# drowe67/radae

Measured on AMD Instinct MI355X. Metric: vocoder-feature frames/sec (enc+chan+dec), model19, higher is better.
Workload: dtype f32 I/O, 2xf16 (22-bit) MFMA operands, f32 accumulate (refine: f64 MFMA)

## Files before the change

### radae_amd/csrc/rade_dev.h

```cpp
#ifndef RADE_DEV_H
#define RADE_DEV_H

#include <stdint.h>

#ifdef __cplusplus
extern "C" {
#endif

#define RD_M        160
#define RD_NCP      32
#define RD_SYM      192
#define RD_NC       30
#define RD_NS       4
#define RD_NMF      960
#define RD_NEOO     1152
#define RD_RXBUF    2112
#define RD_NFC      40
#define RD_NQ       16
#define RD_NTAP     101
#define RD_NINMAX   1120
#define RD_LATENT   80
#define RD_ZMF      240
#define RD_FEAT_MF  432
#define RD_NEOOBITS 180
// ... 94 lines not shown

#define RD_EF_KB   (RD_ENC_W / 16)
#define RD_EF_TILE (RD_EF_KB * 1024)
typedef struct {
    const unsigned short *xf; int NQ;
    int B, T, K0, K1, dil;
    const unsigned short *Wp16; const float *Wscale; const float *bias; int N, act;
    float *y; long y_sb, y_st;
    unsigned short *yf; int ycol;
    int seq_taps, no_pair;
    int pair;
    const float *xin; int Kin; const float *Wp;
} rd_encf_args;
int rd_launch_encf_gemm(const rd_encf_args *a, rd_stream_t s);
int rd_launch_encf_dense1(const rd_encf_args *a, rd_stream_t s);
int rd_launch_encf_hist(unsigned short *xf, int NQ, float *x32, long x32_sb, int B, int T, int dir, rd_stream_t s);

int rd_launch_enc_pack(const float *features, float *xin, int B, int T, rd_stream_t s);
int rd_launch_pad_rows(const float *src, float *dst, long R, int K, int Kpad, rd_stream_t s);
int rd_launch_chan_symbol(const float *z, const float *H, const float *noise, float *out, long n_real, int mode, float p0, float p1, unsigned long long seed, rd_stream_t s);
int rd_launch_carry_rows(float *x, int B, int Tcap, int W, int nhist, int T, const int *n_rows, rd_stream_t s);
int rd_launch_ofdm_mod(const rd_tables *tab, const float *z, void *tx, long tx_stride, int B, int n_mf, int linear, rd_stream_t s);
int rd_launch_ofdm_mod_mp(const rd_tables *tab, const float *z, void *tx, long tx_stride, int B, int n_mf, const void *G, void *mp, double *part, int linear, rd_stream_t s);
int rd_launch_eoo_build(const rd_tables *tab, const float *bits, float *eoo, int B, rd_stream_t s);
int rd_launch_copy_eoo(const float *eoo, void *out, long stride, int B, rd_stream_t s);

enum { RD_IRX_LS = 0, RD_IRX_MEAN6 = 1, RD_IRX_ALL = 2, RD_IRX_NONE = 3 };
typedef struct {
    const rd_tables *tab; const void *rx; long rx_stride;
    const float *foff;
    int n_mf, time_offset, eq, coarse_mag, B;
    float mag_scale;
    float *z_hat;
    double *part;
    const float *z_ref; long long *n_err;
} rd_irx_args;
int rd_launch_irx(const rd_irx_args *a, rd_stream_t s);

// ... 125 lines not shown
```

### radae_amd/csrc/rade_enc.hip

```cpp
#include "rade_devutil.h"

#define EF_TILE RD_EF_TILE

template <bool LIBM_TANH>
__device__ __forceinline__ void encf_emit(const rd_encf_args &a, int b, int t, int ch0, f32x4 v, f32x4 sc, f32x4 bs)
{
#pragma unroll
    for (int c = 0; c < 4; c++) {
        float x = v[c] * sc[c] + bs[c];
        if (a.act == 1) x = clamp1(LIBM_TANH ? tanhf(x) : gate_tanh(x));
        v[c] = x;
    }
    if (a.yf) {
        const int col = a.ycol + ch0;
        _Float16 *o = (_Float16 *)a.yf + ((size_t)b * a.NQ + 1 + (t >> 5)) * EF_TILE + (col >> 4) * 1024 + ((col >> 3) & 1) * 256 + (t & 31) * 8 + (col & 4);
        f16x4 hi, lo;
#pragma unroll
        for (int c = 0; c < 4; c++) { const float x = 256.0f * v[c]; const _Float16 h = (_Float16)x; hi[c] = h; lo[c] = (_Float16)(x - (float)h); }
        *(f16x4 *)o = hi; *(f16x4 *)(o + 512) = lo;
    } else {
        *(f32x4 *)(a.y + (size_t)b * a.y_sb + (size_t)t * a.y_st + ch0) = v;
    }
}

// ... 98 lines not shown
#pragma unroll
        for (int i = 0; i < NT; i++)
#pragma unroll
            for (int g = 0; g < 4; g++) {
                const int ch0 = 32 * (nt0 + i) + 8 * g + 4 * half;
                if (ch0 >= a.N) continue;
                const f32x4 bs = a.bias ? *(const f32x4 *)(a.bias + ch0) : (f32x4){ 0.0f, 0.0f, 0.0f, 0.0f };
                f32x4 sc = { 0x1p-18f, 0x1p-18f, 0x1p-18f, 0x1p-18f };
                if (SINGLE) { sc = *(const f32x4 *)(a.Wscale + ch0); sc *= 0x1p-8f; }
                const f32x4 v = { acc[q][i][4 * g], acc[q][i][4 * g + 1], acc[q][i][4 * g + 2], acc[q][i][4 * g + 3] };
                encf_emit<false>(a, b, t, ch0, v, sc, bs);
            }
    }
}

__global__ __launch_bounds__(64) void k_encf_dense1(rd_encf_args a)
{
    constexpr int NT = 2;
    const int lane = threadIdx.x, r = lane & 31, half = lane >> 5;
    const int tpq = (a.T + 31) >> 5;
    const int b = blockIdx.x / tpq, qt = blockIdx.x - b * tpq;
    const int t = 32 * qt + r;
    const float *p = a.xin + ((size_t)b * a.T + min(t, a.T - 1)) * a.Kin + 4 * half;
    f32x16 acc[NT];
#pragma unroll
    for (int i = 0; i < NT; i++)
#pragma unroll
        for (int j = 0; j < 16; j++) acc[i][j] = 0.0f;
    const float *wp = a.Wp + (size_t)lane * 4;
    const size_t wstep = (size_t)NT * 256;
    const int nkb = a.Kin >> 3;
    f32x4 av = *(const f32x4 *)p;
    f32x4 bv[NT];
#pragma unroll
    for (int i = 0; i < NT; i++) bv[i] = *(const f32x4 *)(wp + i * 256);
    for (int kb = 0; kb < nkb; kb++) {
        f32x4 an = av; f32x4 bn[NT];
#pragma unroll
        for (int i = 0; i < NT; i++) bn[i] = bv[i];
        if (kb + 1 < nkb) {
            an = *(const f32x4 *)(p + (kb + 1) * 8);
#pragma unroll
            for (int i = 0; i < NT; i++) bn[i] = *(const f32x4 *)(wp + wstep + i * 256);
        }
#pragma unroll
        for (int s = 0; s < 4; s++)
#pragma unroll
            for (int i = 0; i < NT; i++)
                acc[i] = __builtin_amdgcn_mfma_f32_32x32x2f32(bv[i][s], av[s], acc[i], 0, 0, 0);
        av = an;
#pragma unroll
        for (int i = 0; i < NT; i++) bv[i] = bn[i];
        wp += wstep;
    }
    if (t >= a.T) return;
#pragma unroll
// ... 43 lines not shown
        }
    }
}

extern "C" int rd_launch_encf_hist(unsigned short *xf, int NQ, float *x32, long x32_sb, int B, int T, int dir, rd_stream_t s)
{
    if (B <= 0) return 0;
    hipLaunchKernelGGL(k_encf_hist, dim3(B), dim3(256), 0, (hipStream_t)s, xf, NQ, x32, x32_sb, T, dir);
    return (int)hipGetLastError();
}

extern "C" int rd_launch_encf_dense1(const rd_encf_args *a, rd_stream_t s)
{
    if (a->B <= 0 || a->T <= 0) return 0;
    if (a->N != 64 || (a->Kin & 7) || !a->yf) return -1;
    hipLaunchKernelGGL(k_encf_dense1, dim3(a->B * ((a->T + 31) >> 5)), dim3(64), 0, (hipStream_t)s, *a);
    return (int)hipGetLastError();
}

extern "C" int rd_launch_encf_gemm(const rd_encf_args *a, rd_stream_t s)
{
    if (a->B <= 0 || a->T <= 0) return 0;
    const int ntt = (a->N + 31) >> 5, tpq = (a->T + 31) >> 5;
    if ((a->K0 & 15) || (a->K1 & 15) || ntt % 3 || (a->N & 3) || a->dil < 0 || a->dil > 2) return -1;
    hipStream_t st = (hipStream_t)s;
    const int seq = a->seq_taps, nopair = a->no_pair;
    rd_encf_args b = *a;
    const int ntile = a->B * tpq;
    b.pair = (ntt == 6 && !nopair) ? 1 : 0;
    const dim3 g = b.pair ? dim3(((ntile + 7) / 8) * 16, 1) : dim3(ntile, ntt / 3), blk(64);
    const bool ti = a->K0 > 0 && a->K0 == a->K1 && !seq;
// ... 9 lines not shown
```

### radae_amd/csrc/rade_engine.c

```c
#define _GNU_SOURCE
#define __HIP_PLATFORM_AMD__ 1
#include <hip/hip_runtime_api.h>

#include <pthread.h>
#include <time.h>
#include <sched.h>
#include <stdio.h>
#include <stdlib.h>
#include <string.h>
#include <stdint.h>
#include <math.h>

#include "rade_batch.h"
#include "rade_api.h"
#include "rade_host.h"

#define CHK(x) do { hipError_t e_ = (x); if (e_ != hipSuccess) { fprintf(stderr, "rade: HIP error %s at %s:%d\n", hipGetErrorString(e_), __FILE__, __LINE__); goto fail; } } while (0)

static int g_engines_open;
double rade_host_cpu_quota(void)
{
    cpu_set_t set; double n = 1.0;
    if (sched_getaffinity(0, sizeof set, &set) == 0) n = (double)CPU_COUNT(&set);
    FILE *f = fopen("/sys/fs/cgroup/cpu.max", "r");
// ... 23 lines not shown

#define ON_DEV(h) do { if (h) (void)hipSetDevice((h)->device); } while (0)

#define RADE_PROF_MAXEV 256
#define RADE_PROF_MAXIV 4096
struct rade_batch {
    struct owned *owned;
    int alloc_failed;
    int B, max_tx_mf, device, flags, trace_cap, Tcap;
    int R, dec_rows;
    int unsync_off_after;
    unsigned short *corrq16, *corra16, *wfwd16, *bpf16; double *vm; int rx_lds, rx_census;
    int feat_in, enc_kpad, bottleneck1;
    float *dec2_x, *dec2_gi, *dec2_hbuf, *dec2_h[5];
    rd_tables *d_tab;
    dev_lin enc_dense1, enc_zdense, dec_dense1, dec_output, enc_gin[5], dec_gin[5], enc_conv[5], dec_conv[5], dec_glu[5];
    float *enc_whh[5], *enc_bhh[5], *dec_whh[5], *dec_bhh[5];
    unsigned short *dec_whq[5]; float *dec_whs[5];
    float *enc_xin, *enc_x, *enc_gi, *enc_h[5], *enc_z, *eoo, *eoo_bits;
    unsigned short *enc_xf; int enc_nq, enc_seq_taps, enc_no_pair;
    int enc_hist_frag;
    int bypass_dec;
    int tx_linear;
    double *irx_part; long irx_part_cap; float *irx_foff; long long *irx_err;
    rd_bpf_state *tx_bpf, *tx_bpf_init; void *tx_raw; float *tx_chain; float *eoo_filt;
    void *chan_scratch; void *chan_mp;
    float *chan_ps, *chan_ps_host;
    float *rs_sigma; double *rs_part, *rs_stats;
    int *loss_len; double *loss_res, *loss_part; long loss_part_cap;
    rd_rx_stream *rx_st; rd_rx_round *rx_round;
// ... 181 lines not shown
    if (h->R < 1) h->R = 1;
    if (h->R > RD_RX_ROUND_MAX) h->R = RD_RX_ROUND_MAX;
    h->dec_rows = getenv("RADE_DEC_ROWS") ? atoi(getenv("RADE_DEC_ROWS")) : 48;
    if (h->dec_rows < 3) h->dec_rows = 3;
    if (h->dec_rows > 63) h->dec_rows = 63;
    const size_t DR = (size_t)h->dec_rows;

    rd_tables *tab = malloc(sizeof *tab);
    rd_tables_fill(tab);
    h->d_tab = dev_upload(h, tab, sizeof *tab);
    h->corrq16 = upload_table16(h, tab, rd_corrq16_table_fill, RD_CORRQ16_HALFS);
    h->corra16 = upload_table16(h, tab, rd_corra16_table_fill, RD_CORRA16_HALFS);
    h->wfwd16 = upload_table16(h, tab, rd_wfwd16_table_fill, RD_WFWD16_HALFS);
    h->bpf16 = upload_table16(h, tab, rd_bpf16_table_fill, RD_BPF16_HALFS);
    free(tab);
    {
        double vm[8][RD_M];
        for (int n = 0; n < RD_M; n++) { const double nu = ((double)n - 79.5) / 80.0; double v = 1.0; for (int m = 0; m < 8; m++) { vm[m][n] = v; v *= nu; } }
        h->vm = dev_upload(h, vm, sizeof vm);
    }
    h->rx_lds = rd_rx_sync_prepare();
    h->rx_census = getenv("RADE_RX2_CENSUS") ? atoi(getenv("RADE_RX2_CENSUS")) : 0;
    if (h->alloc_failed || h->rx_lds <= 0) goto fail;

    int err = 0;
    h->feat_in = m.enc_dense1.n_in; h->enc_kpad = (h->feat_in + 15) & ~15; h->bottleneck1 = (cfg->flags & RADE_BATCH_BOTTLENECK1) != 0;
    err |= upload_lin(h, &h->enc_dense1, m.enc_dense1.w, m.enc_dense1.b, NULL, 64, h->feat_in, h->enc_kpad);
    err |= upload_lin(h, &h->enc_zdense, m.enc_zdense.w, m.enc_zdense.b, NULL, 80, 864, 864);
    err |= upload_lin(h, &h->dec_dense1, m.dec_dense1.w, m.dec_dense1.b, NULL, 96, 80, 80);
    err |= upload_lin(h, &h->dec_output, m.dec_output.w, m.dec_output.b, NULL, h->feat_in, 736, 736);
// ... 65 lines not shown
    h->dec2_gi = dev_zeros(h, sizeof(float) * B * T * 288);
    h->dec2_hbuf = dev_zeros(h, sizeof(float) * B * T * 96);
    h->dtcache = dev_zeros(h, sizeof(float) * B * 2 * RD_NMF * RD_NFC);
    if (h->trace_cap > 0) {
        h->trace = dev_zeros(h, sizeof(rd_rx_trace) * B * h->trace_cap);
        h->trace_z = dev_zeros(h, sizeof(float) * B * h->trace_cap * RD_ZMF);
    }
    h->h_small = must(h, pinned_alloc_opt(h, sizeof(int) * (8 + B * 8)));
    h->lcg_seeds = malloc(sizeof(unsigned) * B);
    for (size_t b = 0; b < B; b++) h->lcg_seeds[b] = 1u;
    h->d_lcg_seeds = dev_upload(h, h->lcg_seeds, sizeof(unsigned) * B);
    if (h->alloc_failed) { fprintf(stderr, "rade: device allocation failed\n"); goto fail; }
    for (int i = 0; i < 2 * RADE_PROF_MAXEV; i++) CHK(hipEventCreate(&h->prof_ev[i]));
    CHK(hipEventCreateWithFlags(&h->ev_block, hipEventBlockingSync | hipEventDisableTiming));
    rade_batch_rx_reset(h);
    if (rd_launch_eoo_build(h->d_tab, NULL, h->eoo, h->B, NULL)) goto fail;
    CHK(hipDeviceSynchronize());
    rd_model_free(&m);
    return h;
fail:
    if (have_model) rd_model_free(&m);
    if (h) rade_batch_close(h);
    return NULL;
}

rade_batch *rade_batch_open(const char *blob_path, const rade_batch_config *cfg)
{
    FILE *f = blob_path ? fopen(blob_path, "rb") : NULL;
    if (!f) { fprintf(stderr, "rade: cannot open weight blob %s\n", blob_path ? blob_path : "(null)"); return NULL; }
    fseek(f, 0, SEEK_END); long n = ftell(f); fseek(f, 0, SEEK_SET);
    void *buf = malloc(n);
// ... 6 lines not shown

void rade_batch_close(rade_batch *h)
{
    if (!h) return;
    ON_DEV(h);
    while (h->owned) disown(h, h->owned->p);
    if (h->ev_block) hipEventDestroy(h->ev_block);
    __atomic_sub_fetch(&g_engines_open, 1, __ATOMIC_RELAXED);
    for (int i = 0; i < 2 * RADE_PROF_MAXEV; i++) if (h->prof_ev[i]) hipEventDestroy(h->prof_ev[i]);
    free(h->lcg_seeds);
    free(h);
}

int rade_batch_n_streams(const rade_batch *h) { return h->B; }
const rd_tables *rd_batch_tables(const rade_batch *h) { return h->d_tab; }
int rd_batch_has_tx_bpf(const rade_batch *h) { return h->tx_bpf != NULL; }

static void prof_drain(rade_batch *h)
{
    for (int i = 0; i < h->prof_cnt; i++) {
        float ms = 0;
        if (hipEventSynchronize(h->prof_ev[2 * i + 1]) == hipSuccess && hipEventElapsedTime(&ms, h->prof_ev[2 * i], h->prof_ev[2 * i + 1]) == hipSuccess) {
            h->prof_ms[h->prof_cls[i]] += ms; h->prof_flops[h->prof_cls[i]] += h->prof_fl[i]; h->prof_n[h->prof_cls[i]]++;
            float t0 = 0;
            if (h->prof_ref && h->iv_n < RADE_PROF_MAXIV && hipEventElapsedTime(&t0, h->prof_ref, h->prof_ev[2 * i]) == hipSuccess) {
                h->iv_cls[h->iv_n] = h->prof_cls[i]; h->iv_t0[h->iv_n] = t0; h->iv_t1[h->iv_n] = t0 + ms; h->iv_n++;
            }
        }
    }
    h->prof_cnt = 0;
// ... 45 lines not shown

static int encf_gemm(rade_batch *h, const dev_lin *w, int K1, int K0, int dil, float *y, long y_sb, long y_st, int ycol, int T, int act, void *stream)
{
    rd_encf_args g;
    memset(&g, 0, sizeof g);
    g.xf = h->enc_xf; g.NQ = h->enc_nq; g.B = h->B; g.T = T; g.K0 = K0; g.K1 = K1; g.dil = dil;
    g.Wp16 = w->wp16; g.Wscale = w->wscale16; g.bias = w->bias; g.N = w->N; g.act = act;
    g.y = y; g.y_sb = y_sb; g.y_st = y_st; if (!y) { g.yf = h->enc_xf; g.ycol = ycol; }
    g.seq_taps = h->enc_seq_taps; g.no_pair = h->enc_no_pair;
    if (K0 + K1 != w->K || !w->wp16) { fprintf(stderr, "rade: internal GEMM shape error (%d+%d != %d)\n", K0, K1, w->K); return -1; }
    PROF_BEGIN(h, stream);
    const int rc = rd_launch_encf_gemm(&g, stream);
    PROF_END(h, stream, RADE_PROF_GEMM, 2.0 * (double)h->B * T * (K0 + K1) * w->N);
    return rc;
}
static int encode_core_frag(rade_batch *h, int T, float *z, void *stream)
{
    const int B = h->B;
    int e = h->enc_hist_frag ? 0 : rd_launch_encf_hist(h->enc_xf, h->enc_nq, h->enc_x, (long)(2 + h->Tcap) * RD_ENC_W, B, T, 0, stream);
    {
        rd_encf_args g;
        memset(&g, 0, sizeof g);
        g.xf = h->enc_xf; g.NQ = h->enc_nq; g.B = B; g.T = T; g.bias = h->enc_dense1.bias; g.N = 64; g.act = 1; g.yf = h->enc_xf; g.ycol = 0;
        g.xin = h->enc_xin; g.Kin = h->enc_kpad; g.Wp = h->enc_dense1.wp;
        PROF_BEGIN(h, stream); e |= rd_launch_encf_dense1(&g, stream); PROF_END(h, stream, RADE_PROF_GEMM, 2.0 * (double)B * T * h->enc_kpad * 64);
    }
    e |= encf_gemm(h, &h->enc_gin[0], ENC_IN[0], 0, 0, h->enc_gi, (long)T * 192, 192, 0, T, 0, stream);
    for (int l = 0; l < 5 && !e; l++) {
        const int in = ENC_IN[l], cin = in + 64;
        rd_scan_args s = { h->enc_gi, (long)T * 192, 192, h->enc_whh[l], h->enc_bhh[l], h->enc_h[l], NULL, 0, 0, NULL, 0, NULL, B, T, 64, h->enc_xf, h->enc_nq, in };
        PROF_BEGIN(h, stream); e |= rd_launch_gru_scan(&s, stream); PROF_END(h, stream, RADE_PROF_SCAN, 2.0 * B * T * 192 * 64);
        e |= encf_gemm(h, &h->enc_conv[l], cin, cin, ENC_DIL[l], NULL, 0, 0, cin, T, 1, stream);
        if (l < 4) e |= encf_gemm(h, &h->enc_gin[l + 1], ENC_IN[l + 1], 0, 0, h->enc_gi, (long)T * 192, 192, 0, T, 0, stream);
        else e |= encf_gemm(h, &h->enc_zdense, 864, 0, 0, z, (long)T * RD_LATENT, RD_LATENT, 0, T, h->bottleneck1 ? 1 : 0, stream);
    }
    e |= rd_launch_encf_hist(h->enc_xf, h->enc_nq, h->enc_x, (long)(2 + h->Tcap) * RD_ENC_W, B, T, 1, stream);
    h->enc_hist_frag = !e;
    return e;
}

static int encode_core(rade_batch *h, int T, float *z, void *stream)
{
    const int B = h->B, W = RD_ENC_W;
    if (h->enc_xf && (long)B * T > 16384) return encode_core_frag(h, T, z, stream);
    h->enc_hist_frag = 0;
    const long xsb = (long)(2 + h->Tcap) * W;
    float *x0 = h->enc_x + 2 * W;
    int e = 0;
    dev_lin d1 = h->enc_dense1; d1.wp16 = NULL; d1.wscale16 = NULL;
    e |= gemm(h, &d1, h->enc_xin, (long)T * h->enc_kpad, h->enc_kpad, h->enc_kpad, NULL, 0, 0, 0, NULL, NULL, x0, xsb, W, B, T, 1, stream);
    for (int l = 0; l < 5 && !e; l++) {
        const int in = ENC_IN[l], cin = in + 64;
        e |= gemm(h, &h->enc_gin[l], x0, xsb, W, in, NULL, 0, 0, 0, NULL, NULL, h->enc_gi, (long)T * 192, 192, B, T, 0, stream);
        rd_scan_args s = { h->enc_gi, (long)T * 192, 192, h->enc_whh[l], h->enc_bhh[l], h->enc_h[l], x0 + in, xsb, W, NULL, 0, NULL, B, T, 64 };
        PROF_BEGIN(h, stream); e |= rd_launch_gru_scan(&s, stream); PROF_END(h, stream, RADE_PROF_SCAN, 2.0 * B * T * 192 * 64);
        e |= gemm(h, &h->enc_conv[l], x0, xsb, W, cin, x0 - (long)ENC_DIL[l] * W, xsb, W, cin, NULL, NULL, x0 + cin, xsb, W, B, T, 1, stream);
    }
    e |= gemm(h, &h->enc_zdense, x0, xsb, W, 864, NULL, 0, 0, 0, NULL, NULL, z, (long)T * RD_LATENT, RD_LATENT, B, T, h->bottleneck1 ? 1 : 0, stream);
    e |= rd_launch_carry_rows(h->enc_x, B, h->Tcap, W, 2, T, NULL, stream);
// ... 3 lines not shown
static int tx_bpf_pass(rade_batch *h, int n, int len0, void *out, long out_stride, void *stream, int advance)
{
    rd_bpf_args ba;
    memset(&ba, 0, sizeof ba);
    ba.state = h->tx_bpf; ba.state_stride = sizeof(rd_bpf_state); ba.len0_const = len0; ba.avail_const = n;
    ba.tab = h->d_tab; ba.bpf16 = h->bpf16; ba.x = h->tx_raw; ba.x_stride = tx_raw_stride(h); ba.y = out; ba.y_stride = out_stride;
    ba.chain = h->tx_chain; ba.chain_stride = h->max_tx_mf + 8; ba.n_blocks = 1 + (n > len0 ? (n - len0 + RD_NMF - 1) / RD_NMF : 0); ba.B = h->B; ba.clip = 1; ba.advance = advance;
    PROF_BEGIN(h, stream);
    const int rc = rd_launch_bpf(&ba, stream);
    PROF_END(h, stream, RADE_PROF_BPF, 8.0 * 101.0 * (double)h->B * n);
    return rc;
}

static int encode_features(rade_batch *h, const float *features_dev, int T, float *z, void *stream)
{
    const int e = rd_launch_enc_pack(features_dev, h->enc_xin, h->B, T, stream);
    return e | encode_core(h, T, z, stream);
}
static int modulate(rade_batch *h, const float *z, int n_mf, void *iq_out, long iq_stride, void *stream)
{
    void *mod_out = h->tx_bpf ? h->tx_raw : iq_out; const long mod_stride = h->tx_bpf ? tx_raw_stride(h) : iq_stride;
    PROF_BEGIN(h, stream);
    int e = rd_launch_ofdm_mod(h->d_tab, z, mod_out, mod_stride, h->B, n_mf, h->tx_linear, stream);
    PROF_END(h, stream, RADE_PROF_MOD, 8.0 * h->B * n_mf * 5 * 30 * 160);
    if (h->tx_bpf) e |= tx_bpf_pass(h, n_mf * RD_NMF, RD_NMF, iq_out, iq_stride, stream, 1);
    return e;
}

int rade_batch_tx(rade_batch *h, const float *features_dev, int n_mf, void *iq_out_dev, long iq_stride, float *z_out_dev, void *stream)
{
    ON_DEV(h);
    if (!h || !features_dev || !iq_out_dev || n_mf <= 0 || n_mf > h->max_tx_mf || h->feat_in != 84) return -1;
    if (misaligned16(z_out_dev)) return -1;
    float *z = z_out_dev ? z_out_dev : h->enc_z;
    int e = encode_features(h, features_dev, 3 * n_mf, z, stream);
    e |= modulate(h, z, n_mf, iq_out_dev, iq_stride, stream);
    return e ? -1 : n_mf * RD_NMF;
}
// ... 119 lines not shown
{
    ON_DEV(h);
    if (!h || !p || n_mf <= 0 || n_mf > h->max_tx_mf || h->feat_in != 84 || p->n_sig != n_mf * RD_NMF || !rx_out_dev || (h->tx_linear && p->with_eoo)) return -1;
    if (!features_dev || misaligned16(p->G_dev)) return -1;
    const float *ps_dev;
    if (chan_streams_upload(h, p, ps, stream, &ps_dev)) return -1;
    if (!p->G_dev || h->tx_bpf) {
        if (!iq_out_dev) return -1;
        if (rade_batch_tx(h, features_dev, n_mf, iq_out_dev, iq_stride, NULL, stream) != p->n_sig) return -1;
        return channel_dev(h, iq_out_dev, iq_stride, rx_out_dev, rx_stride, p, ps_dev, stream);
    }
    if (dev_grow(h, &h->chan_mp, NULL, (long)h->B * h->max_tx_mf * RD_NMF, sizeof(float) * 2, 1)) return -1;
    const int B = h->B;
    int e = encode_features(h, features_dev, 3 * n_mf, h->enc_z, stream);
    PROF_BEGIN(h, stream);
    e |= rd_launch_ofdm_mod_mp(h->d_tab, h->enc_z, iq_out_dev, iq_stride, B, n_mf, p->G_dev, h->chan_mp, (double *)h->chan_scratch + 2 * (size_t)B, h->tx_linear, stream);
    PROF_END(h, stream, RADE_PROF_MOD, 8.0 * B * n_mf * 5 * 30 * 160);
    if (e) return -1;
    return channel_launch(h, p, ps_dev, NULL, 0, h->chan_mp, h->eoo, rx_out_dev, rx_stride, stream);
}

int rade_batch_tx_channel(rade_batch *h, const float *features_dev, int n_mf, void *iq_out_dev, long iq_stride, void *rx_out_dev, long rx_stride,
                          const rade_channel_params *p, void *stream)
{
    return rade_batch_tx_channel_streams(h, features_dev, n_mf, iq_out_dev, iq_stride, rx_out_dev, rx_stride, p, NULL, stream);
}

int rade_batch_multipath_gen(rade_batch *h, const float *fir_taps_host, int n_taps, int low_ratio, int n_out,
                             const void *noise_low_dev, unsigned long long seed, void *G_out_dev, void *stream)
{
    ON_DEV(h);
// ... 311 lines not shown
```

### radae_amd/csrc/rade_host.h

```cpp
#ifndef RADE_HOST_H
#define RADE_HOST_H

#include <stddef.h>

#include "rade_dev.h"

#ifdef __cplusplus
extern "C" {
#endif

typedef struct { int n_in, n_out; float *w, *b; float *row_scale; } rd_linear;
typedef struct { int n_in, hid; float *w_ih, *w_hh, *b_ih, *b_hh; float *s_ih, *s_hh; } rd_gru;

typedef struct {
    rd_linear enc_dense1, enc_zdense, dec_dense1, dec_output;
    rd_gru enc_gru[5], dec_gru[5];
    rd_linear enc_conv[5], dec_conv[5];
    rd_linear dec_glu[5];
} rd_model;

const char *rd_find_default_model(const char *hint, char *buf, size_t n);

void rd_tables_fill(rd_tables *T);
int rd_model_parse(const void *blob, size_t len, rd_model *m);
// ... 12 lines not shown
long rd_pack_weights_f16x2(const float *W, int N, int K, unsigned short *out);
long rd_pack_weights_q16(const float *W, const float *row_scale, int N, int K, unsigned short *out, float *scale_out);
int rd_chunkmajor_q16(const float *W, const float *row_scale, int N, int K, int Kpad, int Npad, unsigned short *out);
void rd_chunkmajor_f32(const float *W, int N, int K, int Kpad, int Npad, float *out);
long rd_packed16a_size(int N, int K);
long rd_pack_weights_q16_a16(const float *W, const float *row_scale, int N, int K, unsigned short *out, float *scale_out);
long rd_pack_weights_f16x2_a16(const float *W, int N, int K, unsigned short *out);
#ifdef __cplusplus
}
#endif
void *rd_core_tx_open(const void *blob, int len, const rd_tables *d_tab);
void rd_core_tx_close(void *t);
int rd_core_tx_frame(void *t, const float *features_in, float *tx_out);
struct rade_batch;
const rd_tables *rd_batch_tables(const struct rade_batch *h);
int rd_batch_has_tx_bpf(const struct rade_batch *h);

#endif
```

### radae_amd/csrc/rade_kernels.hip

```cpp
#include "rade_devutil.h"

__device__ float g_zero_row[2048];

template <int NT>
__global__ __launch_bounds__(64) void k_gemm(rd_gemm_args a)
{
    const int lane = threadIdx.x;
    const int rows = a.B * a.T;
    const int r0 = blockIdx.x * 32;
    const int ntt = (a.N + 31) >> 5;
    const int nt0 = blockIdx.y * NT;
    int r = r0 + (lane & 31);
    if (r >= rows) r = rows - 1;
    const int b = r / a.T, t = r - b * a.T;
    const int half = lane >> 5;
    const float *p1 = a.a1 + b * a.a1_sb + t * a.a1_st + 4 * half;
    const float *p0 = nullptr;
    if (a.K0) {
        const bool rst = a.reset && a.reset[b * a.reset_sb + t];
        p0 = (rst ? g_zero_row : a.a0 + b * a.a0_sb + t * a.a0_st) + 4 * half;
    }
    f32x16 acc[NT];
#pragma unroll
    for (int i = 0; i < NT; i++)
// ... 515 lines not shown
    float v[8];
#pragma unroll
    for (int q = 0; q < 8; q++) { const int i = threadIdx.x + q * 256; v[q] = i < n ? base[(size_t)Tb * W + i] : 0.0f; }
    __syncthreads();
#pragma unroll
    for (int q = 0; q < 8; q++) { const int i = threadIdx.x + q * 256; if (i < n) base[i] = v[q]; }
}
extern "C" int rd_launch_carry_rows(float *x, int B, int Tcap, int W, int nhist, int T, const int *n_rows, rd_stream_t s)
{
    if (B <= 0) return 0;
    hipLaunchKernelGGL(k_carry_rows, dim3(B), dim3(256), 0, (hipStream_t)s, x, Tcap, W, nhist, T, n_rows);
    return (int)hipGetLastError();
}


template <bool LINEAR>
__global__ __launch_bounds__(192) void k_ofdm_mod(const rd_tables *tab, const float *z, float2 *tx, long tx_stride, int n_mf)
{
    __shared__ float2 sym[RD_NS + 1][RD_NC];
    const int mf = blockIdx.x, b = blockIdx.y, tid = threadIdx.x;
    const float *zf = z + ((size_t)b * n_mf + mf) * RD_ZMF;
    const float pg = LINEAR ? 1.0f : tab->pilot_gain;
    if (tid < RD_NC) sym[0][tid] = make_float2(tab->P[tid] * pg, 0.0f * pg);
    if (tid < 120) sym[1 + tid / RD_NC][tid % RD_NC] = make_float2(zf[2 * tid], zf[2 * tid + 1]);
    __syncthreads();
    float2 *out = tx + (size_t)b * tx_stride + (size_t)mf * RD_NMF;
    if (tid < RD_M) {
        f32x2 acc[RD_NS + 1];
#pragma unroll
        for (int s = 0; s <= RD_NS; s++) acc[s] = (f32x2){ 0.0f, 0.0f };
#pragma unroll 6
        for (int c = 0; c < RD_NC; c++) {
            const float2 w = ld2(tab->Winv[c], tid);
#pragma unroll
            for (int s = 0; s <= RD_NS; s++) acc[s] = idft_term(acc[s], sym[s][c], w);
        }
#pragma unroll
        for (int s = 0; s <= RD_NS; s++) {
            const float2 v = LINEAR ? make_float2(acc[s][0], acc[s][1]) : pa_limit(make_float2(acc[s][0], acc[s][1]));
            out[s * RD_SYM + RD_NCP + tid] = v;
            if (tid >= RD_M - RD_NCP) out[s * RD_SYM + tid - (RD_M - RD_NCP)] = v;
        }
    }
}
extern "C" int rd_launch_ofdm_mod(const rd_tables *tab, const float *z, void *tx, long tx_stride, int B, int n_mf, int linear, rd_stream_t s)
{
    if (B <= 0 || n_mf <= 0) return 0;
    if (linear) hipLaunchKernelGGL(k_ofdm_mod<true>, dim3(n_mf, B), dim3(192), 0, (hipStream_t)s, tab, z, (float2 *)tx, tx_stride, n_mf);
    else hipLaunchKernelGGL(k_ofdm_mod<false>, dim3(n_mf, B), dim3(192), 0, (hipStream_t)s, tab, z, (float2 *)tx, tx_stride, n_mf);
    return (int)hipGetLastError();
}

template <bool LINEAR>
__global__ __launch_bounds__(192) void k_ofdm_mod_mp(const rd_tables *tab, const float *z, float2 *tx, long tx_stride, int n_mf, const float2 *G, float2 *mp, double *part)
{
    __shared__ float2 sym[RD_NS + 1][RD_NC];
    __shared__ float2 prevsym[RD_NC];
    __shared__ float2 fr[16 + RD_NMF];
    __shared__ double red[2][4];
    const int mf = blockIdx.x, b = blockIdx.y, tid = threadIdx.x;
    const float *zf = z + ((size_t)b * n_mf + mf) * RD_ZMF;
    const float pg = LINEAR ? 1.0f : tab->pilot_gain;
    if (tid < RD_NC) sym[0][tid] = make_float2(tab->P[tid] * pg, 0.0f * pg);
    if (tid < 120) sym[1 + tid / RD_NC][tid % RD_NC] = make_float2(zf[2 * tid], zf[2 * tid + 1]);
    if (tid >= 128 && tid < 128 + RD_NC && mf > 0) { const int c = tid - 128; prevsym[c] = make_float2(zf[-RD_ZMF + 2 * (90 + c)], zf[-RD_ZMF + 2 * (90 + c) + 1]); }
    __syncthreads();
    if (tid < RD_M) {
        f32x2 acc[RD_NS + 1];
#pragma unroll
        for (int s = 0; s <= RD_NS; s++) acc[s] = (f32x2){ 0.0f, 0.0f };
#pragma unroll 6
        for (int c = 0; c < RD_NC; c++) {
            const float2 w = ld2(tab->Winv[c], tid);
#pragma unroll
            for (int s = 0; s <= RD_NS; s++) acc[s] = idft_term(acc[s], sym[s][c], w);
        }
#pragma unroll
        for (int s = 0; s <= RD_NS; s++) {
            const float2 v = LINEAR ? make_float2(acc[s][0], acc[s][1]) : pa_limit(make_float2(acc[s][0], acc[s][1]));
            fr[16 + s * RD_SYM + RD_NCP + tid] = v;
            if (tid >= RD_M - RD_NCP) fr[16 + s * RD_SYM + tid - (RD_M - RD_NCP)] = v;
        }
    } else if (tid < RD_M + 16) {
        const int n = RD_M - 16 + (tid - RD_M);
        float2 a = make_float2(0.0f, 0.0f);
        if (mf > 0) { f32x2 ac = { 0.0f, 0.0f }; for (int c = 0; c < RD_NC; c++) ac = idft_term(ac, prevsym[c], ld2(tab->Winv[c], n)); a = LINEAR ? make_float2(ac[0], ac[1]) : pa_limit(make_float2(ac[0], ac[1])); }
        fr[tid - RD_M] = a;
    }
    __syncthreads();
    const size_t base = (size_t)mf * RD_NMF;
    const f32x4 *Gb = (const f32x4 *)G + (size_t)b * n_mf * RD_NMF;
    float2 *mpo = mp + (size_t)b * n_mf * RD_NMF + base;
    float2 *txo = tx ? tx + (size_t)b * tx_stride + base : nullptr;
// ... 13 lines not shown
#pragma unroll
    for (int q = 0; q < 5; q++) {
        const int i = tid + 192 * q;
        const float2 x = fr[16 + i];
        const float2 m = cadd(a1[q], c2[i]);
        mpo[i] = m;
        if (txo) txo[i] = x;
        const float ax = hypotf(x.x, x.y), am = hypotf(m.x, m.y);
        s0 += (double)(ax * ax); s1 += (double)(am * am);
    }
    s0 = wave_sum_f64(s0); s1 = wave_sum_f64(s1);
    if ((tid & 63) == 0) { red[0][tid >> 6] = s0; red[1][tid >> 6] = s1; }
    __syncthreads();
    if (tid == 0) { part[((size_t)b * n_mf + mf) * 2] = (red[0][0] + red[0][1]) + red[0][2]; part[((size_t)b * n_mf + mf) * 2 + 1] = (red[1][0] + red[1][1]) + red[1][2]; }
}
extern "C" int rd_launch_ofdm_mod_mp(const rd_tables *tab, const float *z, void *tx, long tx_stride, int B, int n_mf, const void *G, void *mp, double *part, int linear, rd_stream_t s)
{
    if (B <= 0 || n_mf <= 0) return 0;
    if (linear) hipLaunchKernelGGL(k_ofdm_mod_mp<true>, dim3(n_mf, B), dim3(192), 0, (hipStream_t)s, tab, z, (float2 *)tx, tx_stride, n_mf, (const float2 *)G, (float2 *)mp, part);
    else hipLaunchKernelGGL(k_ofdm_mod_mp<false>, dim3(n_mf, B), dim3(192), 0, (hipStream_t)s, tab, z, (float2 *)tx, tx_stride, n_mf, (const float2 *)G, (float2 *)mp, part);
    return (int)hipGetLastError();
}

__global__ __launch_bounds__(192) void k_eoo_build(const rd_tables *tab, const float *bits, float2 *eoo)
{
    __shared__ float2 sym[RD_NS - 1][RD_NC];
    const int b = blockIdx.x, tid = threadIdx.x;
    float2 *out = eoo + (size_t)b * RD_NEOO;
    for (int i = tid; i < RD_NEOO; i += blockDim.x) out[i] = ld2(tab->eoo, i);
    if (!bits) return;
    if (tid < 90) sym[tid / RD_NC][tid % RD_NC] = make_float2(bits[b * RD_NEOOBITS + 2 * tid], bits[b * RD_NEOOBITS + 2 * tid + 1]);
    __syncthreads();
    if (tid < RD_M) {
        for (int s = 0; s < RD_NS - 1; s++) {
            float2 acc = make_float2(0.0f, 0.0f);
// ... 245 lines not shown
```

Before: 85.67 million.

## Precompute constant pilot symbol and fuse feature packing into encoder dense1

Computes the pilot OFDM symbol once at init into a device table, so the modulator kernels copy it instead of recomputing one of five IDFT symbols per modem frame. Separately, the encoder dense1 kernel gains a FEAT variant that reads the raw feature rows directly and builds the padded input on the fly, which removes the separate enc_pack kernel and its intermediate buffer for large batches. Both paths can be turned off with an environment variable. The risks are the on-the-fly index arithmetic in the GEMM A-load and less coalesced feature reads.

```diff
diff --git a/radae_amd/csrc/rade_dev.h b/radae_amd/csrc/rade_dev.h
--- a/radae_amd/csrc/rade_dev.h
+++ b/radae_amd/csrc/rade_dev.h
@@ -132,14 +132,16 @@
 } rd_encf_args;
 int rd_launch_encf_gemm(const rd_encf_args *a, rd_stream_t s);
 int rd_launch_encf_dense1(const rd_encf_args *a, rd_stream_t s);
+int rd_launch_encf_dense1_feat(const rd_encf_args *a, rd_stream_t s);
 int rd_launch_encf_hist(unsigned short *xf, int NQ, float *x32, long x32_sb, int B, int T, int dir, rd_stream_t s);
 
 int rd_launch_enc_pack(const float *features, float *xin, int B, int T, rd_stream_t s);
 int rd_launch_pad_rows(const float *src, float *dst, long R, int K, int Kpad, rd_stream_t s);
 int rd_launch_chan_symbol(const float *z, const float *H, const float *noise, float *out, long n_real, int mode, float p0, float p1, unsigned long long seed, rd_stream_t s);
 int rd_launch_carry_rows(float *x, int B, int Tcap, int W, int nhist, int T, const int *n_rows, rd_stream_t s);
-int rd_launch_ofdm_mod(const rd_tables *tab, const float *z, void *tx, long tx_stride, int B, int n_mf, int linear, rd_stream_t s);
-int rd_launch_ofdm_mod_mp(const rd_tables *tab, const float *z, void *tx, long tx_stride, int B, int n_mf, const void *G, void *mp, double *part, int linear, rd_stream_t s);
+int rd_launch_pilot_sym(const rd_tables *tab, float *pilot, rd_stream_t s);
+int rd_launch_ofdm_mod(const rd_tables *tab, const float *pilot, const float *z, void *tx, long tx_stride, int B, int n_mf, int linear, rd_stream_t s);
+int rd_launch_ofdm_mod_mp(const rd_tables *tab, const float *pilot, const float *z, void *tx, long tx_stride, int B, int n_mf, const void *G, void *mp, double *part, int linear, rd_stream_t s);
 int rd_launch_eoo_build(const rd_tables *tab, const float *bits, float *eoo, int B, rd_stream_t s);
 int rd_launch_copy_eoo(const float *eoo, void *out, long stride, int B, rd_stream_t s);
 
diff --git a/radae_amd/csrc/rade_enc.hip b/radae_amd/csrc/rade_enc.hip
--- a/radae_amd/csrc/rade_enc.hip
+++ b/radae_amd/csrc/rade_enc.hip
@@ -136,6 +136,7 @@
     }
 }
 
+template <bool FEAT>
 __global__ __launch_bounds__(64) void k_encf_dense1(rd_encf_args a)
 {
     constexpr int NT = 2;
@@ -143,7 +144,19 @@
     const int tpq = (a.T + 31) >> 5;
     const int b = blockIdx.x / tpq, qt = blockIdx.x - b * tpq;
     const int t = 32 * qt + r;
-    const float *p = a.xin + ((size_t)b * a.T + min(t, a.T - 1)) * a.Kin + 4 * half;
+    const float *p = FEAT ? a.xin + ((size_t)b * a.T + min(t, a.T - 1)) * (4 * 36) : a.xin + ((size_t)b * a.T + min(t, a.T - 1)) * a.Kin + 4 * half;
+    auto lda = [&](int kb) -> f32x4 {
+        if (!FEAT) return *(const f32x4 *)(p + kb * 8);
+        f32x4 v;
+#pragma unroll
+        for (int s = 0; s < 4; s++) {
+            const int c = 8 * kb + 4 * half + s, fr = c / 21, j = c - 21 * fr;
+            const bool data = c < 84 && j < 20;
+            const float x = p[data ? fr * 36 + j : 0];
+            v[s] = data ? x : (c < 84 ? -1.0f : 0.0f);
+        }
+        return v;
+    };
     f32x16 acc[NT];
 #pragma unroll
     for (int i = 0; i < NT; i++)
@@ -152,7 +165,7 @@
     const float *wp = a.Wp + (size_t)lane * 4;
     const size_t wstep = (size_t)NT * 256;
     const int nkb = a.Kin >> 3;
-    f32x4 av = *(const f32x4 *)p;
+    f32x4 av = lda(0);
     f32x4 bv[NT];
 #pragma unroll
     for (int i = 0; i < NT; i++) bv[i] = *(const f32x4 *)(wp + i * 256);
@@ -161,7 +174,7 @@
 #pragma unroll
         for (int i = 0; i < NT; i++) bn[i] = bv[i];
         if (kb + 1 < nkb) {
-            an = *(const f32x4 *)(p + (kb + 1) * 8);
+            an = lda(kb + 1);
 #pragma unroll
             for (int i = 0; i < NT; i++) bn[i] = *(const f32x4 *)(wp + wstep + i * 256);
         }
@@ -235,7 +248,14 @@
 {
     if (a->B <= 0 || a->T <= 0) return 0;
     if (a->N != 64 || (a->Kin & 7) || !a->yf) return -1;
-    hipLaunchKernelGGL(k_encf_dense1, dim3(a->B * ((a->T + 31) >> 5)), dim3(64), 0, (hipStream_t)s, *a);
+    hipLaunchKernelGGL(k_encf_dense1<false>, dim3(a->B * ((a->T + 31) >> 5)), dim3(64), 0, (hipStream_t)s, *a);
+    return (int)hipGetLastError();
+}
+extern "C" int rd_launch_encf_dense1_feat(const rd_encf_args *a, rd_stream_t s)
+{
+    if (a->B <= 0 || a->T <= 0) return 0;
+    if (a->N != 64 || a->Kin != RD_ENC_IN || !a->yf) return -1;
+    hipLaunchKernelGGL(k_encf_dense1<true>, dim3(a->B * ((a->T + 31) >> 5)), dim3(64), 0, (hipStream_t)s, *a);
     return (int)hipGetLastError();
 }
 
diff --git a/radae_amd/csrc/rade_engine.c b/radae_amd/csrc/rade_engine.c
--- a/radae_amd/csrc/rade_engine.c
+++ b/radae_amd/csrc/rade_engine.c
@@ -61,6 +61,8 @@
     int feat_in, enc_kpad, bottleneck1;
     float *dec2_x, *dec2_gi, *dec2_hbuf, *dec2_h[5];
     rd_tables *d_tab;
+    float *pilot_tab;
+    int tx_unfused;
     dev_lin enc_dense1, enc_zdense, dec_dense1, dec_output, enc_gin[5], dec_gin[5], enc_conv[5], dec_conv[5], dec_glu[5];
     float *enc_whh[5], *enc_bhh[5], *dec_whh[5], *dec_bhh[5];
     unsigned short *dec_whq[5]; float *dec_whs[5];
@@ -272,6 +274,8 @@
     h->wfwd16 = upload_table16(h, tab, rd_wfwd16_table_fill, RD_WFWD16_HALFS);
     h->bpf16 = upload_table16(h, tab, rd_bpf16_table_fill, RD_BPF16_HALFS);
     free(tab);
+    h->pilot_tab = dev_zeros(h, sizeof(float) * 2 * 2 * RD_SYM);
+    h->tx_unfused = getenv("RADE_TX_UNFUSED") ? atoi(getenv("RADE_TX_UNFUSED")) : 0;
     {
         double vm[8][RD_M];
         for (int n = 0; n < RD_M; n++) { const double nu = ((double)n - 79.5) / 80.0; double v = 1.0; for (int m = 0; m < 8; m++) { vm[m][n] = v; v *= nu; } }
@@ -367,7 +371,7 @@
     for (int i = 0; i < 2 * RADE_PROF_MAXEV; i++) CHK(hipEventCreate(&h->prof_ev[i]));
     CHK(hipEventCreateWithFlags(&h->ev_block, hipEventBlockingSync | hipEventDisableTiming));
     rade_batch_rx_reset(h);
-    if (rd_launch_eoo_build(h->d_tab, NULL, h->eoo, h->B, NULL)) goto fail;
+    if (rd_launch_eoo_build(h->d_tab, NULL, h->eoo, h->B, NULL) || rd_launch_pilot_sym(h->d_tab, h->pilot_tab, NULL)) goto fail;
     CHK(hipDeviceSynchronize());
     rd_model_free(&m);
     return h;
@@ -404,6 +408,12 @@
 
 int rade_batch_n_streams(const rade_batch *h) { return h->B; }
 const rd_tables *rd_batch_tables(const rade_batch *h) { return h->d_tab; }
+int rd_batch_pilot_symbol(const rade_batch *h, int linear, float *out)
+{
+    ON_DEV(h);
+    return hipMemcpy(out, h->pilot_tab + (linear ? 2 * RD_SYM : 0), sizeof(float) * 2 * RD_SYM, hipMemcpyDeviceToHost) == hipSuccess ? 0 : -1;
+}
+static const float *pilot_tab(const rade_batch *h) { return (h->tx_unfused & 1) ? NULL : h->pilot_tab; }
 int rd_batch_has_tx_bpf(const rade_batch *h) { return h->tx_bpf != NULL; }
 
 static void prof_drain(rade_batch *h)
@@ -479,7 +489,7 @@
     PROF_END(h, stream, RADE_PROF_GEMM, 2.0 * (double)h->B * T * (K0 + K1) * w->N);
     return rc;
 }
-static int encode_core_frag(rade_batch *h, int T, float *z, void *stream)
+static int encode_core_frag(rade_batch *h, const float *feat, int T, float *z, void *stream)
 {
     const int B = h->B;
     int e = h->enc_hist_frag ? 0 : rd_launch_encf_hist(h->enc_xf, h->enc_nq, h->enc_x, (long)(2 + h->Tcap) * RD_ENC_W, B, T, 0, stream);
@@ -487,8 +497,8 @@
         rd_encf_args g;
         memset(&g, 0, sizeof g);
         g.xf = h->enc_xf; g.NQ = h->enc_nq; g.B = B; g.T = T; g.bias = h->enc_dense1.bias; g.N = 64; g.act = 1; g.yf = h->enc_xf; g.ycol = 0;
-        g.xin = h->enc_xin; g.Kin = h->enc_kpad; g.Wp = h->enc_dense1.wp;
-        PROF_BEGIN(h, stream); e |= rd_launch_encf_dense1(&g, stream); PROF_END(h, stream, RADE_PROF_GEMM, 2.0 * (double)B * T * h->enc_kpad * 64);
+        g.xin = feat ? feat : h->enc_xin; g.Kin = h->enc_kpad; g.Wp = h->enc_dense1.wp;
+        PROF_BEGIN(h, stream); e |= feat ? rd_launch_encf_dense1_feat(&g, stream) : rd_launch_encf_dense1(&g, stream); PROF_END(h, stream, RADE_PROF_GEMM, 2.0 * (double)B * T * h->enc_kpad * 64);
     }
     e |= encf_gemm(h, &h->enc_gin[0], ENC_IN[0], 0, 0, h->enc_gi, (long)T * 192, 192, 0, T, 0, stream);
     for (int l = 0; l < 5 && !e; l++) {
@@ -504,10 +514,11 @@
     return e;
 }
 
+static int enc_takes_frag(const rade_batch *h, int T) { return h->enc_xf && (long)h->B * T > 16384; }
 static int encode_core(rade_batch *h, int T, float *z, void *stream)
 {
     const int B = h->B, W = RD_ENC_W;
-    if (h->enc_xf && (long)B * T > 16384) return encode_core_frag(h, T, z, stream);
+    if (enc_takes_frag(h, T)) return encode_core_frag(h, NULL, T, z, stream);
     h->enc_hist_frag = 0;
     const long xsb = (long)(2 + h->Tcap) * W;
     float *x0 = h->enc_x + 2 * W;
@@ -541,6 +552,7 @@
 
 static int encode_features(rade_batch *h, const float *features_dev, int T, float *z, void *stream)
 {
+    if (enc_takes_frag(h, T) && h->enc_kpad == RD_ENC_IN && !(h->tx_unfused & 2)) return encode_core_frag(h, features_dev, T, z, stream);
     const int e = rd_launch_enc_pack(features_dev, h->enc_xin, h->B, T, stream);
     return e | encode_core(h, T, z, stream);
 }
@@ -548,7 +560,7 @@
 {
     void *mod_out = h->tx_bpf ? h->tx_raw : iq_out; const long mod_stride = h->tx_bpf ? tx_raw_stride(h) : iq_stride;
     PROF_BEGIN(h, stream);
-    int e = rd_launch_ofdm_mod(h->d_tab, z, mod_out, mod_stride, h->B, n_mf, h->tx_linear, stream);
+    int e = rd_launch_ofdm_mod(h->d_tab, pilot_tab(h), z, mod_out, mod_stride, h->B, n_mf, h->tx_linear, stream);
     PROF_END(h, stream, RADE_PROF_MOD, 8.0 * h->B * n_mf * 5 * 30 * 160);
     if (h->tx_bpf) e |= tx_bpf_pass(h, n_mf * RD_NMF, RD_NMF, iq_out, iq_stride, stream, 1);
     return e;
@@ -698,7 +710,7 @@
     const int B = h->B;
     int e = encode_features(h, features_dev, 3 * n_mf, h->enc_z, stream);
     PROF_BEGIN(h, stream);
-    e |= rd_launch_ofdm_mod_mp(h->d_tab, h->enc_z, iq_out_dev, iq_stride, B, n_mf, p->G_dev, h->chan_mp, (double *)h->chan_scratch + 2 * (size_t)B, h->tx_linear, stream);
+    e |= rd_launch_ofdm_mod_mp(h->d_tab, pilot_tab(h), h->enc_z, iq_out_dev, iq_stride, B, n_mf, p->G_dev, h->chan_mp, (double *)h->chan_scratch + 2 * (size_t)B, h->tx_linear, stream);
     PROF_END(h, stream, RADE_PROF_MOD, 8.0 * B * n_mf * 5 * 30 * 160);
     if (e) return -1;
     return channel_launch(h, p, ps_dev, NULL, 0, h->chan_mp, h->eoo, rx_out_dev, rx_stride, stream);
diff --git a/radae_amd/csrc/rade_host.h b/radae_amd/csrc/rade_host.h
--- a/radae_amd/csrc/rade_host.h
+++ b/radae_amd/csrc/rade_host.h
@@ -50,6 +50,7 @@
 int rd_core_tx_frame(void *t, const float *features_in, float *tx_out);
 struct rade_batch;
 const rd_tables *rd_batch_tables(const struct rade_batch *h);
+int rd_batch_pilot_symbol(const struct rade_batch *h, int linear, float *out);
 int rd_batch_has_tx_bpf(const struct rade_batch *h);
 
 #endif
diff --git a/radae_amd/csrc/rade_kernels.hip b/radae_amd/csrc/rade_kernels.hip
--- a/radae_amd/csrc/rade_kernels.hip
+++ b/radae_amd/csrc/rade_kernels.hip
@@ -553,46 +553,75 @@
 }
 
 
-template <bool LINEAR>
-__global__ __launch_bounds__(192) void k_ofdm_mod(const rd_tables *tab, const float *z, float2 *tx, long tx_stride, int n_mf)
-{
+__global__ __launch_bounds__(192) void k_pilot_sym(const rd_tables *tab, float2 *pil)
+{
+    __shared__ float2 sym[RD_NC];
+    const int lin = blockIdx.x, tid = threadIdx.x;
+    const float pg = lin ? 1.0f : tab->pilot_gain;
+    if (tid < RD_NC) sym[tid] = make_float2(tab->P[tid] * pg, 0.0f * pg);
+    __syncthreads();
+    float2 *out = pil + lin * RD_SYM;
+    if (tid < RD_M) {
+        f32x2 acc = { 0.0f, 0.0f };
+        for (int c = 0; c < RD_NC; c++) acc = idft_term(acc, sym[c], ld2(tab->Winv[c], tid));
+        const float2 v = lin ? make_float2(acc[0], acc[1]) : pa_limit(make_float2(acc[0], acc[1]));
+        out[RD_NCP + tid] = v;
+        if (tid >= RD_M - RD_NCP) out[tid - (RD_M - RD_NCP)] = v;
+    }
+}
+extern "C" int rd_launch_pilot_sym(const rd_tables *tab, float *pilot, rd_stream_t s)
+{
+    hipLaunchKernelGGL(k_pilot_sym, dim3(2), dim3(192), 0, (hipStream_t)s, tab, (float2 *)pilot);
+    return (int)hipGetLastError();
+}
+
+template <bool LINEAR, bool PTAB>
+__global__ __launch_bounds__(192) void k_ofdm_mod(const rd_tables *tab, const float2 *pil, const float *z, float2 *tx, long tx_stride, int n_mf)
+{
+    constexpr int S0 = PTAB ? 1 : 0;
     __shared__ float2 sym[RD_NS + 1][RD_NC];
     const int mf = blockIdx.x, b = blockIdx.y, tid = threadIdx.x;
     const float *zf = z + ((size_t)b * n_mf + mf) * RD_ZMF;
     const float pg = LINEAR ? 1.0f : tab->pilot_gain;
-    if (tid < RD_NC) sym[0][tid] = make_float2(tab->P[tid] * pg, 0.0f * pg);
+    if (!PTAB && tid < RD_NC) sym[0][tid] = make_float2(tab->P[tid] * pg, 0.0f * pg);
     if (tid < 120) sym[1 + tid / RD_NC][tid % RD_NC] = make_float2(zf[2 * tid], zf[2 * tid + 1]);
     __syncthreads();
     float2 *out = tx + (size_t)b * tx_stride + (size_t)mf * RD_NMF;
+    if (PTAB) out[tid] = pil[tid];
     if (tid < RD_M) {
         f32x2 acc[RD_NS + 1];
 #pragma unroll
-        for (int s = 0; s <= RD_NS; s++) acc[s] = (f32x2){ 0.0f, 0.0f };
+        for (int s = S0; s <= RD_NS; s++) acc[s] = (f32x2){ 0.0f, 0.0f };
 #pragma unroll 6
         for (int c = 0; c < RD_NC; c++) {
             const float2 w = ld2(tab->Winv[c], tid);
 #pragma unroll
-            for (int s = 0; s <= RD_NS; s++) acc[s] = idft_term(acc[s], sym[s][c], w);
-        }
-#pragma unroll
-        for (int s = 0; s <= RD_NS; s++) {
+            for (int s = S0; s <= RD_NS; s++) acc[s] = idft_term(acc[s], sym[s][c], w);
+        }
+#pragma unroll
+        for (int s = S0; s <= RD_NS; s++) {
             const float2 v = LINEAR ? make_float2(acc[s][0], acc[s][1]) : pa_limit(make_float2(acc[s][0], acc[s][1]));
             out[s * RD_SYM + RD_NCP + tid] = v;
             if (tid >= RD_M - RD_NCP) out[s * RD_SYM + tid - (RD_M - RD_NCP)] = v;
         }
     }
 }
-extern "C" int rd_launch_ofdm_mod(const rd_tables *tab, const float *z, void *tx, long tx_stride, int B, int n_mf, int linear, rd_stream_t s)
+extern "C" int rd_launch_ofdm_mod(const rd_tables *tab, const float *pilot, const float *z, void *tx, long tx_stride, int B, int n_mf, int linear, rd_stream_t s)
 {
     if (B <= 0 || n_mf <= 0) return 0;
-    if (linear) hipLaunchKernelGGL(k_ofdm_mod<true>, dim3(n_mf, B), dim3(192), 0, (hipStream_t)s, tab, z, (float2 *)tx, tx_stride, n_mf);
-    else hipLaunchKernelGGL(k_ofdm_mod<false>, dim3(n_mf, B), dim3(192), 0, (hipStream_t)s, tab, z, (float2 *)tx, tx_stride, n_mf);
-    return (int)hipGetLastError();
-}
-
-template <bool LINEAR>
-__global__ __launch_bounds__(192) void k_ofdm_mod_mp(const rd_tables *tab, const float *z, float2 *tx, long tx_stride, int n_mf, const float2 *G, float2 *mp, double *part)
-{
+    const float2 *pil = pilot ? (const float2 *)pilot + (linear ? RD_SYM : 0) : nullptr;
+    const dim3 g(n_mf, B), blk(192);
+    if (linear && pil) hipLaunchKernelGGL((k_ofdm_mod<true, true>), g, blk, 0, (hipStream_t)s, tab, pil, z, (float2 *)tx, tx_stride, n_mf);
+    else if (linear) hipLaunchKernelGGL((k_ofdm_mod<true, false>), g, blk, 0, (hipStream_t)s, tab, pil, z, (float2 *)tx, tx_stride, n_mf);
+    else if (pil) hipLaunchKernelGGL((k_ofdm_mod<false, true>), g, blk, 0, (hipStream_t)s, tab, pil, z, (float2 *)tx, tx_stride, n_mf);
+    else hipLaunchKernelGGL((k_ofdm_mod<false, false>), g, blk, 0, (hipStream_t)s, tab, pil, z, (float2 *)tx, tx_stride, n_mf);
+    return (int)hipGetLastError();
+}
+
+template <bool LINEAR, bool PTAB>
+__global__ __launch_bounds__(192) void k_ofdm_mod_mp(const rd_tables *tab, const float2 *pil, const float *z, float2 *tx, long tx_stride, int n_mf, const float2 *G, float2 *mp, double *part)
+{
+    constexpr int S0 = PTAB ? 1 : 0;
     __shared__ float2 sym[RD_NS + 1][RD_NC];
     __shared__ float2 prevsym[RD_NC];
     __shared__ float2 fr[16 + RD_NMF];
@@ -600,22 +629,23 @@
     const int mf = blockIdx.x, b = blockIdx.y, tid = threadIdx.x;
     const float *zf = z + ((size_t)b * n_mf + mf) * RD_ZMF;
     const float pg = LINEAR ? 1.0f : tab->pilot_gain;
-    if (tid < RD_NC) sym[0][tid] = make_float2(tab->P[tid] * pg, 0.0f * pg);
+    if (!PTAB && tid < RD_NC) sym[0][tid] = make_float2(tab->P[tid] * pg, 0.0f * pg);
     if (tid < 120) sym[1 + tid / RD_NC][tid % RD_NC] = make_float2(zf[2 * tid], zf[2 * tid + 1]);
     if (tid >= 128 && tid < 128 + RD_NC && mf > 0) { const int c = tid - 128; prevsym[c] = make_float2(zf[-RD_ZMF + 2 * (90 + c)], zf[-RD_ZMF + 2 * (90 + c) + 1]); }
     __syncthreads();
+    if (PTAB) fr[16 + tid] = pil[tid];
     if (tid < RD_M) {
         f32x2 acc[RD_NS + 1];
 #pragma unroll
-        for (int s = 0; s <= RD_NS; s++) acc[s] = (f32x2){ 0.0f, 0.0f };
+        for (int s = S0; s <= RD_NS; s++) acc[s] = (f32x2){ 0.0f, 0.0f };
 #pragma unroll 6
         for (int c = 0; c < RD_NC; c++) {
             const float2 w = ld2(tab->Winv[c], tid);
 #pragma unroll
-            for (int s = 0; s <= RD_NS; s++) acc[s] = idft_term(acc[s], sym[s][c], w);
-        }
-#pragma unroll
-        for (int s = 0; s <= RD_NS; s++) {
+            for (int s = S0; s <= RD_NS; s++) acc[s] = idft_term(acc[s], sym[s][c], w);
+        }
+#pragma unroll
+        for (int s = S0; s <= RD_NS; s++) {
             const float2 v = LINEAR ? make_float2(acc[s][0], acc[s][1]) : pa_limit(make_float2(acc[s][0], acc[s][1]));
             fr[16 + s * RD_SYM + RD_NCP + tid] = v;
             if (tid >= RD_M - RD_NCP) fr[16 + s * RD_SYM + tid - (RD_M - RD_NCP)] = v;
@@ -659,11 +689,17 @@
     __syncthreads();
     if (tid == 0) { part[((size_t)b * n_mf + mf) * 2] = (red[0][0] + red[0][1]) + red[0][2]; part[((size_t)b * n_mf + mf) * 2 + 1] = (red[1][0] + red[1][1]) + red[1][2]; }
 }
-extern "C" int rd_launch_ofdm_mod_mp(const rd_tables *tab, const float *z, void *tx, long tx_stride, int B, int n_mf, const void *G, void *mp, double *part, int linear, rd_stream_t s)
+extern "C" int rd_launch_ofdm_mod_mp(const rd_tables *tab, const float *pilot, const float *z, void *tx, long tx_stride, int B, int n_mf, const void *G, void *mp, double *part, int linear, rd_stream_t s)
 {
     if (B <= 0 || n_mf <= 0) return 0;
-    if (linear) hipLaunchKernelGGL(k_ofdm_mod_mp<true>, dim3(n_mf, B), dim3(192), 0, (hipStream_t)s, tab, z, (float2 *)tx, tx_stride, n_mf, (const float2 *)G, (float2 *)mp, part);
-    else hipLaunchKernelGGL(k_ofdm_mod_mp<false>, dim3(n_mf, B), dim3(192), 0, (hipStream_t)s, tab, z, (float2 *)tx, tx_stride, n_mf, (const float2 *)G, (float2 *)mp, part);
+    const float2 *pil = pilot ? (const float2 *)pilot + (linear ? RD_SYM : 0) : nullptr;
+    const dim3 g(n_mf, B), blk(192);
+#define MOD_MP(L, P) hipLaunchKernelGGL((k_ofdm_mod_mp<L, P>), g, blk, 0, (hipStream_t)s, tab, pil, z, (float2 *)tx, tx_stride, n_mf, (const float2 *)G, (float2 *)mp, part)
+    if (linear && pil) MOD_MP(true, true);
+    else if (linear) MOD_MP(true, false);
+    else if (pil) MOD_MP(false, true);
+    else MOD_MP(false, false);
+#undef MOD_MP
     return (int)hipGetLastError();
 }
 
```

Result: no change. 85.65 million, median of 2 (-0.0%).
